# castorini/dhr

Hardware: AMD Instinct MI355X
Metric: queries/sec (exact top-1000, brute-force dense-hybrid GIP retrieval) (higher is better)
Workload: dtype i8 (bound GEMM: gated AND ungated columns int8 x int8 -> int32 on the matrix cores, every gated rounding upward, the ungated quantisation error paid by the filter margin) + f64-accumulated f16 x f32 exact rescoring of the survivors -- the returned scores are the exact scores rounded once, identical

## Files before the change

dhr_amd/csrc/gemm_g8.h:

```cpp
#pragma once
#include "gemm_common.h"
#include <climits>

namespace dhr {

typedef int intx4 __attribute__((ext_vector_type(4)));
typedef int intx8 __attribute__((ext_vector_type(8)));

constexpr int G8_QOFF = 16384;
constexpr int G8_SLOT = 32768;
constexpr int G8_META = 4 * G8_SLOT;
constexpr int G8_RING_LDS = 4 * G8_SLOT + 4096 + 64;
constexpr int G8_NT = 512;


__device__ __forceinline__ void g8_smfmac(floatx16& c, const intx4& a, const intx8& b, uint32_t idx) {
  asm("v_smfmac_i32_32x32x64_i8 %0, %1, %2, %3" : "+v"(c) : "v"(a), "v"(b), "v"(idx));
}
__device__ __forceinline__ void g8_mfma(floatx16& c, const intx4& a, const intx4& b) {
  asm("v_mfma_i32_32x32x32_i8 %0, %1, %2, %0" : "+v"(c) : "v"(a), "v"(b));
}

struct G8Frag {
  intx4 a[4];
  intx4 pw;
  union { intx8 v; intx4 h[2]; } b[2];
};

__device__ __forceinline__ int g8_thr_units(float thr, float mul) {
  const float x = thr / mul;
  if (!(x < 2.1e9f)) return INT_MAX;
  if (x < -2.1e9f) return INT_MIN;
  return (int)floorf(x - fabsf(x) * 1e-6f) - 1;
}
__device__ __forceinline__ float g8_score(int sum, float mul) {
  const float x = (float)sum * mul;
  return x + fabsf(x) * 2.4e-7f;
}


hipError_t launch_gemm_g8p(const GemmArgs& a, hipStream_t s);
bool gemm_g8p_ok(const GemmArgs& a);

}
```

dhr_amd/csrc/gemm_g8.hip:

```cpp
#include "gemm_g8.h"
#include <mutex>
#include <type_traits>

#ifndef G8_TRACE
#define G8_TRACE 0
#endif
#ifndef G8_ABL
#define G8_ABL 0
#endif
namespace dhr {

#if G8_TRACE
constexpr int G8_TRACE_SLOTS = 1 << 18;
__device__ unsigned long long g8_trace_buf[G8_TRACE_SLOTS * 8];
__device__ unsigned int g8_trace_n;
#define G8_T(i) do { if (threadIdx.x == 0 && tslot < G8_TRACE_SLOTS) g8_trace_buf[(size_t)tslot * 8 + (i)] = __builtin_readcyclecounter(); } while (0)
#else
#define G8_T(i) do { } while (0)
#endif
__device__ __forceinline__ void g8_dump_tile(const GemmArgs& p, floatx16 (&acc)[4][2], int64_t dt, int qt, int wm, int wn, int lane,
                                             const float (&mul_r)[2]) {
  const int fhalf = lane >> 5;
  const int64_t row_base = dt * TILE_ROWS + wm * 128;
#pragma unroll
  for (int ni = 0; ni < 2; ++ni) {
    const int q = qt * TILE_ROWS + wn * 64 + ni * 32 + (lane & 31);
    if (q < p.n_queries) {
#pragma unroll
      for (int mi = 0; mi < 4; ++mi)
#pragma unroll
        for (int e = 0; e < 16; ++e) {
          const int64_t row = row_base + mi * 32 + (e & 3) + 8 * (e >> 2) + 4 * fhalf;
          if (row < p.n_rows && row >= p.dump_row0 && row - p.dump_row0 < p.dump_ld)
            p.dump[(int64_t)q * p.dump_ld + (row - p.dump_row0)] = g8_score(__float_as_int(acc[mi][ni][e]), mul_r[ni]);
        }
    }
  }
}

template <bool SURPLUS, int NI_, bool CHECK_ROWS = true>
__device__ __forceinline__ void g8_scan_half(const GemmArgs& p, floatx16 (&acc)[4][2], int qt, int wm, int wn, int lane, int rows_valid, int64_t row0,
                                             uint2* stack, const int t, const float mul, uint32_t& j) {
  const int fhalf = lane >> 5;
  const int rbase = wm * 128 + 4 * fhalf;
  const int q = qt * TILE_ROWS + wn * 64 + NI_ * 32 + (lane & 31);
#pragma unroll
  for (int mi = 0; mi < 4; ++mi) {
    const floatx16& a = acc[mi][NI_];
#pragma unroll
    for (int g = 0; g < 4; ++g) {
      const int gm = max(max(__float_as_int(a[4 * g]), __float_as_int(a[4 * g + 1])), max(__float_as_int(a[4 * g + 2]), __float_as_int(a[4 * g + 3])));
      if (gm >= t) {
        asm volatile("");
        if constexpr (!SURPLUS && !CHECK_ROWS) {
#pragma unroll
          for (int e = 4 * g; e < 4 * g + 4; ++e) {
            const int v = __float_as_int(a[e]);
            const int rl = rbase + mi * 32 + (e & 3) + 8 * (e >> 2);
            const uint32_t slot = j < (uint32_t)EPI_STACK ? j : (uint32_t)EPI_STACK;
            stack[slot * G8_NT] = make_uint2((uint32_t)rl, (uint32_t)v);
            j += v >= t ? 1u : 0u;
          }
        } else
#pragma unroll
        for (int e = 4 * g; e < 4 * g + 4; ++e) {
          const int v = __float_as_int(a[e]);
          const int rl = rbase + mi * 32 + (e & 3) + 8 * (e >> 2);
          if (v >= t && (!CHECK_ROWS || rl < rows_valid)) {
            asm volatile("");
            if constexpr (SURPLUS) {
              if (j >= EPI_STACK) {
                const uint32_t slot = atomicAdd(p.cnt + q, 1u);
                cand_store(p, q, slot, make_uint2((uint32_t)(row0 + rl), __float_as_uint(g8_score(v, mul))));
              }
            } else if (j < EPI_STACK) stack[j * G8_NT] = make_uint2((uint32_t)rl, (uint32_t)v);
            ++j;
          }
        }
      }
    }
  }
}
__device__ __forceinline__ void g8_epilogue_surplus(const GemmArgs& p, floatx16 (&acc)[4][2], int qt, int wm, int wn, int lane, int rows_valid, int64_t row0,
                                                 const int (&thr_r)[2], const float (&mul_r)[2]) {
  uint32_t j = 0;
  g8_scan_half<true, 0>(p, acc, qt, wm, wn, lane, rows_valid, row0, nullptr, thr_r[0], mul_r[0], j);
  g8_scan_half<true, 1>(p, acc, qt, wm, wn, lane, rows_valid, row0, nullptr, thr_r[1], mul_r[1], j);
}
__device__ __forceinline__ void g8_epilogue(const GemmArgs& p, floatx16 (&acc)[4][2], int64_t dt, int qt, int wm, int wn, int tid, int lane,
                                            char* smem, const int (&thr_r)[2], const float (&mul_r)[2]) {
  __syncthreads();
  const int64_t row0 = dt * TILE_ROWS;
  const int rows_valid = (int)(p.n_rows - row0 < TILE_ROWS ? p.n_rows - row0 : TILE_ROWS);
  uint2* stack = (uint2*)smem + tid;
  const int q0 = qt * TILE_ROWS + wn * 64 + (lane & 31);
  const bool full = rows_valid == TILE_ROWS;
  uint32_t j = 0;
  if (full) g8_scan_half<false, 0, false>(p, acc, qt, wm, wn, lane, rows_valid, row0, stack, thr_r[0], mul_r[0], j);
  else g8_scan_half<false, 0, true>(p, acc, qt, wm, wn, lane, rows_valid, row0, stack, thr_r[0], mul_r[0], j);
  const uint32_t s0 = j < (uint32_t)EPI_STACK ? j : (uint32_t)EPI_STACK;
#if G8_ABL != 16
  uint32_t base0 = 0u, base1 = 0u;
  if (s0 > 0) base0 = atomicAdd(p.cnt + q0, s0);
#endif
  if (full) g8_scan_half<false, 1, false>(p, acc, qt, wm, wn, lane, rows_valid, row0, stack, thr_r[1], mul_r[1], j);
  else g8_scan_half<false, 1, true>(p, acc, qt, wm, wn, lane, rows_valid, row0, stack, thr_r[1], mul_r[1], j);
  const uint32_t s1 = j < (uint32_t)EPI_STACK ? j : (uint32_t)EPI_STACK;
#if G8_ABL == 16
  return;
#else
  if (s1 > s0) base1 = atomicAdd(p.cnt + q0 + 32, s1 - s0);
  if (__builtin_amdgcn_ballot_w64(j > (uint32_t)EPI_STACK) != 0) g8_epilogue_surplus(p, acc, qt, wm, wn, lane, rows_valid, row0, thr_r, mul_r);
  for (uint32_t i = 0; i < s0; ++i) {
    const uint2 en = stack[i * G8_NT];
    const uint32_t slot = base0 + i;
    cand_store(p, q0, slot, make_uint2((uint32_t)row0 + en.x, __float_as_uint(g8_score((int)en.y, mul_r[0]))));
  }
  for (uint32_t i = s0; i < s1; ++i) {
    const uint2 en = stack[i * G8_NT];
    const uint32_t slot = base1 + (i - s0);
    cand_store(p, q0 + 32, slot, make_uint2((uint32_t)row0 + en.x, __float_as_uint(g8_score((int)en.y, mul_r[1]))));
  }
#endif
}

#if G8_ABL == 2
#define G8_PAIR_SYNC() do { asm volatile("s_waitcnt lgkmcnt(0)" ::: "memory"); __builtin_amdgcn_s_barrier(); } while (0)
#elif G8_ABL == 3
#define G8_PAIR_SYNC() do { asm volatile("s_waitcnt lgkmcnt(0)" ::: "memory"); } while (0)
#else
#define G8_PAIR_SYNC() do { asm volatile("s_waitcnt vmcnt(0) lgkmcnt(0)" ::: "memory"); __builtin_amdgcn_s_barrier(); } while (0)
#endif

#ifndef G8_DMA_SCHED
#define G8_DMA_SCHED 1
#endif
#if G8_DMA_SCHED == 1
__host__ __device__ constexpr int g8_dma_piece(int ph, int g) { return ph == 0 ? g : -1; }
#elif G8_DMA_SCHED == 2
__host__ __device__ constexpr int g8_dma_piece(int ph, int g) { return ph == 0 ? (g >= 2 ? g - 2 : -1) : (ph == 1 && g < 2) ? 6 + g : -1; }
#else
__host__ __device__ constexpr int g8_dma_piece(int ph, int g) { return (ph <= 1 && (g & 1)) ? ph * 4 + (g >> 1) : -1; }
#endif

template <bool DUMP, bool PARTIAL>
__device__ __forceinline__ void g8_tile(const GemmArgs& p, char* smem, const int64_t dt, const int qt, const unsigned tslot = 0) {
  const int lane = threadIdx.x & 63;
  const int wave = __builtin_amdgcn_readfirstlane(threadIdx.x >> 6);
  const int ts = p.ts, td = p.td;
  const int nsp = ts >> 1, npairs = (ts + td) >> 1;
  const char* a_src = (const char*)p.a_tiles + dt * ((int64_t)ts * S8_STAGE_A + (int64_t)td * SP_DENSE);
  const char* b_src = (const char*)p.b_tiles + (int64_t)qt * ((int64_t)ts * SP_STAGE_B + (int64_t)td * SP_DENSE);
  const int wm = PARTIAL ? (wave & 1) : (wave >> 2), wn = PARTIAL ? (wave >> 1) : (wave & 3);
  const bool active = !PARTIAL || wn < p.partial_wn;

  const bool dma_b = ((wave >> 1) & 1) != 0;
  const int dma_s = wave >> 2;
  const int dma_h = wave & 1;
  const uint32_t lane_off = (uint32_t)lane * 16u;
  const uint32_t smem_u = (uint32_t)(uintptr_t)LDS_PTR(smem);
  const __amdgpu_buffer_rsrc_t role_rsrc = __builtin_amdgcn_make_buffer_rsrc((void*)(dma_b ? b_src : a_src), (short)0, 0x7fffffff, 0x00020000);
  int dma_soff = 0, dma_n = 0, nx_soff = 0, nx_n = 0;
  uint32_t dma_lds = 0, nx_lds = 0;
  auto dma_prepare = [&](int g) __attribute__((always_inline)) {
    const int u = 2 * g + dma_s;
    const bool sp = u < ts;
    const int half_bytes = dma_h * ((!dma_b && sp) ? S8_STAGE_A / 2 : 8192);
    if (dma_b) nx_soff = (sp ? u * SP_STAGE_B : ts * SP_STAGE_B + (u - ts) * SP_DENSE) + half_bytes;
    else nx_soff = (sp ? u * S8_STAGE_A : ts * S8_STAGE_A + (u - ts) * SP_DENSE) + half_bytes;
    nx_lds = smem_u + (uint32_t)((u & 3) * G8_SLOT + (dma_b ? G8_QOFF : 0) + half_bytes);
    nx_n = g < npairs ? ((!dma_b && sp) ? 5 : 8) : 0;
    if ((G8_ABL == 4 || G8_ABL == 8) && g >= 2) nx_n = 0;
  };
  auto dma_commit = [&]() __attribute__((always_inline)) { dma_soff = nx_soff; dma_lds = nx_lds; dma_n = nx_n; };
  auto dma_piece = [&](int j) __attribute__((always_inline)) {
    if (j < dma_n) {
      __attribute__((address_space(3))) void* l = (__attribute__((address_space(3))) void*)(uintptr_t)(dma_lds + (uint32_t)(j >> 2) * 4096u);
      const int so = dma_soff + (j >> 2) * 4096;
      switch (j & 3) {
        case 0: __builtin_amdgcn_raw_ptr_buffer_load_lds(role_rsrc, l, 16, (int)lane_off, so, 0, 0); break;
        case 1: __builtin_amdgcn_raw_ptr_buffer_load_lds(role_rsrc, l, 16, (int)lane_off, so, 1024, 0); break;
        case 2: __builtin_amdgcn_raw_ptr_buffer_load_lds(role_rsrc, l, 16, (int)lane_off, so, 2048, 0); break;
        default: __builtin_amdgcn_raw_ptr_buffer_load_lds(role_rsrc, l, 16, (int)lane_off, so, 3072, 0); break;
      }
    }
  };
  auto issue_pair = [&](int g) {
    dma_prepare(g);
    dma_commit();
#pragma unroll
    for (int j = 0; j < 8; ++j) dma_piece(j);
  };

  floatx16 acc[4][2];
  const int frow = lane & 31;
  const int fhalf = lane >> 5;
  const int swz4 = (frow >> 2) & 3;
  const int c0 = (fhalf ^ swz4) << 4, c1 = ((2 + fhalf) ^ swz4) << 4;
  const int a8_off = ((wm * 8 + fhalf) * 32 + frow) * 16;
  const int p8_off = S8_A_BYTES + ((wm * 2 + fhalf) * 32 + frow) * 16;
  const int ad_row = (wm * 128 + frow) * 64;
  const int q_row = G8_QOFF + (wn * 64 + frow) * 64;

  auto read_s8 = [&](G8Frag& f, const char* sl, int g) __attribute__((always_inline)) {
    if (g < 4) f.b[g >> 1].h[g & 1] = *(const intx4*)(sl + q_row + (g >> 1) * 2048 + ((g & 1) ? c1 : c0));
    else if (g < 8) f.a[g - 4] = *(const intx4*)(sl + a8_off + (g - 4) * 1024);
    else if (g == 8) f.pw = *(const intx4*)(sl + p8_off);
  };
  auto read_dn = [&](G8Frag& f, const char* sl, int cc, int g) __attribute__((always_inline)) {
    if (g < 2) f.b[g].h[0] = *(const intx4*)(sl + q_row + g * 2048 + cc);
    else if (g < 6) f.a[g - 2] = *(const intx4*)(sl + ad_row + (g - 2) * 2048 + cc);
  };
  auto blk_s8 = [&](const G8Frag& fc, G8Frag& fn, int un, bool do_load, auto ph_c) __attribute__((always_inline)) {
    constexpr int PH = decltype(ph_c)::value;
    const char* sl = smem + (un & 3) * G8_SLOT;
#pragma unroll
    for (int g = 0; g < 8; ++g) {
      const int ni = g >> 2, mi = g & 3;
      if (!PARTIAL || active) {
        if (do_load && G8_ABL != 8) {
          read_s8(fn, sl, g);
          if (g == 0) read_s8(fn, sl, 8);
        }
        g8_smfmac(acc[mi][ni], fc.a[mi], fc.b[ni].v, (uint32_t)fc.pw[mi]);
      }
      if (g8_dma_piece(PH, g) >= 0) dma_piece(g8_dma_piece(PH, g));
      __builtin_amdgcn_sched_barrier(0);
    }
  };
  auto blk_dn = [&](const G8Frag& fc, G8Frag& fn, int tn, bool do_load, auto ph_c) __attribute__((always_inline)) {
    constexpr int PH = decltype(ph_c)::value;
    const char* sl = smem + ((ts + (tn >> 1)) & 3) * G8_SLOT;
    const int cc = (tn & 1) ? c1 : c0;
#pragma unroll
    for (int g = 0; g < 8; ++g) {
      const int ni = g >> 2, mi = g & 3;
      if (!PARTIAL || active) {
        if (do_load && G8_ABL != 8) read_dn(fn, sl, cc, g);
        g8_mfma(acc[mi][ni], fc.a[mi], fc.b[ni].h[0]);
      }
      if (g8_dma_piece(PH, g) >= 0) dma_piece(g8_dma_piece(PH, g));
      __builtin_amdgcn_sched_barrier(0);
    }
  };

  if (wave < 4 && (ts > 0 || wave == 1 || wave == 2)) {
    const char* src = wave == 0 ? (const char*)(p.g8_rsum + dt * TILE_ROWS) : wave == 1 ? (const char*)(p.i8_mul + qt * TILE_ROWS)
                    : wave == 2 ? (const char*)(p.thr + qt * TILE_ROWS) : (const char*)(p.g8_shift + qt * TILE_ROWS);
    __builtin_amdgcn_global_load_lds(GLOBAL_PTR(src + lane_off), LDS_PTR(smem + G8_META + wave * 1024), 16, 0, 0);
  }
  issue_pair(0);
  if (npairs > 1) {
    issue_pair(1);
    if (dma_n == 5) asm volatile("s_waitcnt vmcnt(5)" ::: "memory"); else asm volatile("s_waitcnt vmcnt(8)" ::: "memory");
  } else asm volatile("s_waitcnt vmcnt(0)" ::: "memory");
  __builtin_amdgcn_s_barrier();
  G8_T(2);
  if (ts > 0) {
    const int32_t* rs = (const int32_t*)(smem + G8_META) + wm * 128 + 4 * (lane >> 5);
#pragma unroll
    for (int mi = 0; mi < 4; ++mi)
#pragma unroll
      for (int g4 = 0; g4 < 4; ++g4) {
        const intx4 v = *(const intx4*)(rs + mi * 32 + 8 * g4);
#pragma unroll
        for (int i4 = 0; i4 < 4; ++i4) acc[mi][0][4 * g4 + i4] = acc[mi][1][4 * g4 + i4] = __int_as_float(v[i4]);
      }
  } else {
#pragma unroll
    for (int mi = 0; mi < 4; ++mi)
#pragma unroll
      for (int e = 0; e < 16; ++e) acc[mi][0][e] = acc[mi][1][e] = 0.f;
  }
  int sh_r[2];
  float mul_r[2], thr_f[2];
#pragma unroll
  for (int ni = 0; ni < 2; ++ni) {
    const int ql = wn * 64 + ni * 32 + (lane & 31);
    mul_r[ni] = ((const float*)(smem + G8_META + 1024))[ql];
    thr_f[ni] = ((const float*)(smem + G8_META + 2048))[ql];
    sh_r[ni] = ts > 0 ? ((const int*)(smem + G8_META + 3072))[ql] : 0;
    asm volatile("" : "+v"(mul_r[ni]), "+v"(thr_f[ni]), "+v"(sh_r[ni]));
  }
  G8Frag f0, f1;
  if (ts > 0) {
#pragma unroll
    for (int g = 0; g < 9; ++g) read_s8(f0, smem, g);
  }
  if (G8_ABL == 8) f1 = f0;
  constexpr std::integral_constant<int, 0> PH0{};
  constexpr std::integral_constant<int, 1> PH1{};
  constexpr std::integral_constant<int, 2> PH2{};
  dma_n = 0;
#pragma unroll 1
  for (int g = 0; g + 1 < nsp; ++g) {
    blk_s8(f0, f1, 2 * g + 1, true, PH1);
    dma_prepare(g + 2);
    __builtin_amdgcn_sched_barrier(0);
    G8_PAIR_SYNC();
    dma_commit();
    blk_s8(f1, f0, 2 * g + 2, true, PH0);
  }
  if (nsp > 0) {
    const int g = nsp - 1;
    blk_s8(f0, f1, 2 * g + 1, true, PH1);
    dma_prepare(g + 2);
    __builtin_amdgcn_sched_barrier(0);
    G8_PAIR_SYNC();
    dma_commit();
    blk_s8(f1, f0, 2 * g + 2, false, PH0);
  }
  G8_T(3);
  if (td > 0) {
    __builtin_amdgcn_sched_barrier(0);
    asm volatile("s_waitcnt lgkmcnt(0)\n\ts_nop 15\n\ts_nop 7" ::: "memory");
    __builtin_amdgcn_sched_barrier(0);
    if (ts > 0)
#pragma unroll
    for (int mi = 0; mi < 4; ++mi)
#pragma unroll
      for (int ni = 0; ni < 2; ++ni)
#pragma unroll
        for (int e = 0; e < 16; ++e) acc[mi][ni][e] = __uint_as_float(__float_as_uint(acc[mi][ni][e]) << sh_r[ni]);
    __builtin_amdgcn_sched_barrier(0);
    {
      const char* sl = smem + (ts & 3) * G8_SLOT;
#pragma unroll
      for (int g = 0; g < 6; ++g) read_dn(f0, sl, c0, g);
    }
    asm volatile("s_nop 4" ::: "memory");
    __builtin_amdgcn_sched_barrier(0);
#pragma unroll 1
    for (int g = nsp; g + 1 < npairs; ++g) {
      const int t0 = 4 * (g - nsp);
      blk_dn(f0, f1, t0 + 1, true, PH1);
      blk_dn(f1, f0, t0 + 2, true, PH2);
      blk_dn(f0, f1, t0 + 3, true, PH2);
      dma_prepare(g + 2);
      __builtin_amdgcn_sched_barrier(0);
      G8_PAIR_SYNC();
      dma_commit();
      blk_dn(f1, f0, t0 + 4, true, PH0);
    }
    {
      const int g = npairs - 1;
      const int t0 = 4 * (g - nsp);
      blk_dn(f0, f1, t0 + 1, true, PH1);
      blk_dn(f1, f0, t0 + 2, true, PH2);
      blk_dn(f0, f1, t0 + 3, true, PH2);
      dma_prepare(g + 2);
      __builtin_amdgcn_sched_barrier(0);
      G8_PAIR_SYNC();
      dma_commit();
      blk_dn(f1, f0, t0 + 4, false, PH0);
    }
  }
  G8_T(4);
  asm volatile("s_waitcnt vmcnt(0) lgkmcnt(0)\n\ts_nop 15\n\ts_nop 7" ::: "memory");
  G8_T(5);
  if (DUMP) { g8_dump_tile(p, acc, dt, qt, wm, wn, lane, mul_r); return; }
  int thr_r[2];
#pragma unroll
  for (int ni = 0; ni < 2; ++ni) {
    asm volatile("" : "+v"(thr_f[ni]));
    thr_r[ni] = g8_thr_units(thr_f[ni], mul_r[ni]);
  }
#if G8_ABL == 32
  if (p.n_queries >= 0) { if (__float_as_int(acc[0][0][0]) == 0x7fffffff) p.cnt[0] = 1; return; }
#endif
  if (PARTIAL && !active) { __syncthreads(); return; }
  g8_epilogue(p, acc, dt, qt, wm, wn, (int)threadIdx.x, lane, smem, thr_r, mul_r);
}

#define G8_KERNEL_ATTR __attribute__((amdgpu_waves_per_eu(2, 2)))
template <bool DUMP>
__global__ void __launch_bounds__(G8_NT) G8_KERNEL_ATTR gemm_filter_g8_kernel(GemmArgs p) {
  extern __shared__ __attribute__((aligned(16))) char smem[];
  int64_t dt;
  int qt;
  if (!gemm_wg_tile(p, dt, qt)) return;
#if G8_TRACE
  unsigned tslot = 0;
  if (threadIdx.x == 0) tslot = atomicAdd(&g8_trace_n, 1u);
  tslot = __builtin_amdgcn_readfirstlane(tslot);
  if (threadIdx.x == 0 && tslot < G8_TRACE_SLOTS) {
    unsigned hw, xcc;
    asm volatile("s_getreg_b32 %0, hwreg(HW_REG_HW_ID)" : "=s"(hw));
    asm volatile("s_getreg_b32 %0, hwreg(HW_REG_XCC_ID)" : "=s"(xcc));
    g8_trace_buf[(size_t)tslot * 8 + 0] = __builtin_amdgcn_s_memrealtime();
    g8_trace_buf[(size_t)tslot * 8 + 7] = (unsigned long long)hw | ((unsigned long long)(xcc & 0xf) << 32) | ((unsigned long long)qt << 40) | ((unsigned long long)(dt & 0xffff) << 48);
  }
  G8_T(1);
  if (!DUMP && p.partial_wn > 0 && qt == p.n_qtiles - 1) g8_tile<false, true>(p, smem, dt, qt, tslot);
  else g8_tile<DUMP, false>(p, smem, dt, qt, tslot);
  G8_T(6);
#else
  if (!DUMP && p.partial_wn > 0 && qt == p.n_qtiles - 1) g8_tile<false, true>(p, smem, dt, qt);
  else g8_tile<DUMP, false>(p, smem, dt, qt);
#endif
}
#if G8_TRACE
}
extern "C" int dhr_debug_g8_trace(unsigned long long* out, int max_slots, unsigned* n_out) try {
  unsigned n = 0;
  if (hipMemcpyFromSymbol(&n, HIP_SYMBOL(dhr::g8_trace_n), 4) != hipSuccess) return -1;
  if (n_out) *n_out = n;
  const unsigned m = n < (unsigned)max_slots ? n : (unsigned)max_slots;
  const unsigned mm = m < (unsigned)dhr::G8_TRACE_SLOTS ? m : (unsigned)dhr::G8_TRACE_SLOTS;
  if (out && mm && hipMemcpyFromSymbol(out, HIP_SYMBOL(dhr::g8_trace_buf), (size_t)mm * 64) != hipSuccess) return -1;
  const unsigned zero = 0;
  if (hipMemcpyToSymbol(HIP_SYMBOL(dhr::g8_trace_n), &zero, 4) != hipSuccess) return -1;
  return 0;
} DHR_CATCH_STATUS
namespace dhr {
#endif

hipError_t launch_gemm_g8(const GemmArgs& a, dim3 grid, hipStream_t s) {
  static std::mutex attr_mu;
  static bool attr_set_dev[64] = {};
  int dev_ = 0;
  (void)hipGetDevice(&dev_);
  {
    std::lock_guard<std::mutex> attr_lock(attr_mu);
    bool& attr_set = attr_set_dev[dev_ & 63];
    if (!attr_set) {
      hipError_t e = hipFuncSetAttribute((const void*)gemm_filter_g8_kernel<false>, hipFuncAttributeMaxDynamicSharedMemorySize, G8_RING_LDS);
      if (e != hipSuccess) return e;
      e = hipFuncSetAttribute((const void*)gemm_filter_g8_kernel<true>, hipFuncAttributeMaxDynamicSharedMemorySize, G8_RING_LDS);
      if (e != hipSuccess) return e;
      attr_set = true;
    }
  }
  if (a.dump) { hipLaunchKernelGGL(gemm_filter_g8_kernel<true>, grid, dim3(G8_NT), G8_RING_LDS, s, a); return hipGetLastError(); }
  GemmArgs b = a;
  constexpr int partial_on = 1;
  const int valid_last = a.n_queries - (a.n_qtiles - 1) * TILE_ROWS;
  b.partial_wn = (partial_on && valid_last > 0 && valid_last <= 128) ? (valid_last + 63) / 64 : 0;
  hipLaunchKernelGGL(gemm_filter_g8_kernel<false>, grid, dim3(G8_NT), G8_RING_LDS, s, b);
  return hipGetLastError();
}

}
```

Baseline: 61680.

## Stage whole above-threshold accumulator groups in LDS with a bitmask for candidate emission

New measurement: 61970, median of 6. About the same (+0.5%).

```diff
diff --git a/dhr_amd/csrc/gemm_g8.h b/dhr_amd/csrc/gemm_g8.h
--- a/dhr_amd/csrc/gemm_g8.h
+++ b/dhr_amd/csrc/gemm_g8.h
@@ -12,6 +12,8 @@
 constexpr int G8_META = 4 * G8_SLOT;
 constexpr int G8_RING_LDS = 4 * G8_SLOT + 4096 + 64;
 constexpr int G8_NT = 512;
+constexpr int G8_GSTACK = 15;
+static_assert((G8_GSTACK + 1) * 16 * G8_NT <= 4 * G8_SLOT, "the group stacks live in the staging ring");
 
 
 __device__ __forceinline__ void g8_smfmac(floatx16& c, const intx4& a, const intx8& b, uint32_t idx) {
diff --git a/dhr_amd/csrc/gemm_g8.hip b/dhr_amd/csrc/gemm_g8.hip
--- a/dhr_amd/csrc/gemm_g8.hip
+++ b/dhr_amd/csrc/gemm_g8.hip
@@ -14,9 +14,16 @@
 constexpr int G8_TRACE_SLOTS = 1 << 18;
 __device__ unsigned long long g8_trace_buf[G8_TRACE_SLOTS * 8];
 __device__ unsigned int g8_trace_n;
-#define G8_T(i) do { if (threadIdx.x == 0 && tslot < G8_TRACE_SLOTS) g8_trace_buf[(size_t)tslot * 8 + (i)] = __builtin_readcyclecounter(); } while (0)
-#else
-#define G8_T(i) do { } while (0)
+#define G8_STAMP(i) do { if (threadIdx.x == 0 && tslot < G8_TRACE_SLOTS) g8_trace_buf[(size_t)tslot * 8 + (i)] = __builtin_readcyclecounter(); } while (0)
+#else
+#define G8_STAMP(i) do { } while (0)
+#endif
+#if G8_TRACE == 2
+#define G8_T(i) do { if ((i) != 3 && (i) != 4) G8_STAMP(i); } while (0)
+#define G8_TE(i) G8_STAMP(i)
+#else
+#define G8_T(i) G8_STAMP(i)
+#define G8_TE(i) do { } while (0)
 #endif
 __device__ __forceinline__ void g8_dump_tile(const GemmArgs& p, floatx16 (&acc)[4][2], int64_t dt, int qt, int wm, int wn, int lane,
                                              const float (&mul_r)[2]) {
@@ -38,12 +45,8 @@
   }
 }
 
-template <bool SURPLUS, int NI_, bool CHECK_ROWS = true>
-__device__ __forceinline__ void g8_scan_half(const GemmArgs& p, floatx16 (&acc)[4][2], int qt, int wm, int wn, int lane, int rows_valid, int64_t row0,
-                                             uint2* stack, const int t, const float mul, uint32_t& j) {
-  const int fhalf = lane >> 5;
-  const int rbase = wm * 128 + 4 * fhalf;
-  const int q = qt * TILE_ROWS + wn * 64 + NI_ * 32 + (lane & 31);
+template <int NI_>
+__device__ __forceinline__ void g8_scan_half(floatx16 (&acc)[4][2], intx4* stack, const int t, uint32_t& jg, uint32_t& mask) {
 #pragma unroll
   for (int mi = 0; mi < 4; ++mi) {
     const floatx16& a = acc[mi][NI_];
@@ -52,74 +55,107 @@
       const int gm = max(max(__float_as_int(a[4 * g]), __float_as_int(a[4 * g + 1])), max(__float_as_int(a[4 * g + 2]), __float_as_int(a[4 * g + 3])));
       if (gm >= t) {
         asm volatile("");
-        if constexpr (!SURPLUS && !CHECK_ROWS) {
-#pragma unroll
-          for (int e = 4 * g; e < 4 * g + 4; ++e) {
-            const int v = __float_as_int(a[e]);
-            const int rl = rbase + mi * 32 + (e & 3) + 8 * (e >> 2);
-            const uint32_t slot = j < (uint32_t)EPI_STACK ? j : (uint32_t)EPI_STACK;
-            stack[slot * G8_NT] = make_uint2((uint32_t)rl, (uint32_t)v);
-            j += v >= t ? 1u : 0u;
-          }
-        } else
-#pragma unroll
-        for (int e = 4 * g; e < 4 * g + 4; ++e) {
-          const int v = __float_as_int(a[e]);
-          const int rl = rbase + mi * 32 + (e & 3) + 8 * (e >> 2);
-          if (v >= t && (!CHECK_ROWS || rl < rows_valid)) {
-            asm volatile("");
-            if constexpr (SURPLUS) {
-              if (j >= EPI_STACK) {
-                const uint32_t slot = atomicAdd(p.cnt + q, 1u);
-                cand_store(p, q, slot, make_uint2((uint32_t)(row0 + rl), __float_as_uint(g8_score(v, mul))));
-              }
-            } else if (j < EPI_STACK) stack[j * G8_NT] = make_uint2((uint32_t)rl, (uint32_t)v);
-            ++j;
+        const uint32_t slot = jg < (uint32_t)G8_GSTACK ? jg : (uint32_t)G8_GSTACK;
+        intx4 v;
+        v[0] = __float_as_int(a[4 * g]); v[1] = __float_as_int(a[4 * g + 1]); v[2] = __float_as_int(a[4 * g + 2]); v[3] = __float_as_int(a[4 * g + 3]);
+        stack[slot * G8_NT] = v;
+        ++jg;
+        mask |= 1u << (NI_ * 16 + mi * 4 + g);
+      }
+    }
+  }
+}
+typedef uint32_t g8_u32x2 __attribute__((ext_vector_type(2)));
+__device__ __forceinline__ void g8_cand_store(const GemmArgs& p, int q, uint32_t slot, uint32_t row, uint32_t score_bits) {
+  g8_u32x2 v;
+  v[0] = row; v[1] = score_bits;
+  typedef __attribute__((address_space(1))) g8_u32x2* gptr;
+  if (slot < p.cap) *(gptr)(uintptr_t)(p.cand + (int64_t)q * p.cap + slot) = v;
+  else if (p.tier) {
+    const ListTier* t = p.tier;
+    const uint32_t o = slot - p.cap;
+    if (o < t->ovf_cap[q]) *(gptr)(uintptr_t)(t->ovf + (size_t)t->ovf_off[q] + o) = v;
+  }
+}
+__device__ __forceinline__ int g8_group_row(int b, int rbase) { return rbase + ((b >> 2) & 3) * 32 + (b & 3) * 8; }
+
+__device__ __forceinline__ void g8_epilogue_surplus(const GemmArgs& p, floatx16 (&acc)[4][2], int q0, int rbase, int rows_valid, int64_t row0,
+                                                    const int (&thr_r)[2], const float (&mul_r)[2], uint32_t mask) {
+#pragma unroll
+  for (int ni = 0; ni < 2; ++ni)
+#pragma unroll
+    for (int mi = 0; mi < 4; ++mi)
+#pragma unroll
+      for (int g = 0; g < 4; ++g) {
+        const int b = ni * 16 + mi * 4 + g;
+        if (b < G8_GSTACK) continue;
+        if (((mask >> b) & 1u) && __popc(mask & ((1u << b) - 1u)) >= G8_GSTACK) {
+#pragma unroll
+          for (int e = 0; e < 4; ++e) {
+            const int v = __float_as_int(acc[mi][ni][4 * g + e]);
+            const int rl = g8_group_row(b, rbase) + e;
+            if (v >= thr_r[ni] && rl < rows_valid) {
+              const uint32_t slot = atomicAdd(p.cnt + q0 + 32 * ni, 1u);
+              cand_store(p, q0 + 32 * ni, slot, make_uint2((uint32_t)(row0 + rl), __float_as_uint(g8_score(v, mul_r[ni]))));
+            }
           }
         }
       }
-    }
-  }
-}
-__device__ __forceinline__ void g8_epilogue_surplus(const GemmArgs& p, floatx16 (&acc)[4][2], int qt, int wm, int wn, int lane, int rows_valid, int64_t row0,
-                                                 const int (&thr_r)[2], const float (&mul_r)[2]) {
-  uint32_t j = 0;
-  g8_scan_half<true, 0>(p, acc, qt, wm, wn, lane, rows_valid, row0, nullptr, thr_r[0], mul_r[0], j);
-  g8_scan_half<true, 1>(p, acc, qt, wm, wn, lane, rows_valid, row0, nullptr, thr_r[1], mul_r[1], j);
 }
 __device__ __forceinline__ void g8_epilogue(const GemmArgs& p, floatx16 (&acc)[4][2], int64_t dt, int qt, int wm, int wn, int tid, int lane,
-                                            char* smem, const int (&thr_r)[2], const float (&mul_r)[2]) {
+                                            char* smem, const int (&thr_r)[2], const float (&mul_r)[2], const unsigned tslot) {
   __syncthreads();
   const int64_t row0 = dt * TILE_ROWS;
   const int rows_valid = (int)(p.n_rows - row0 < TILE_ROWS ? p.n_rows - row0 : TILE_ROWS);
-  uint2* stack = (uint2*)smem + tid;
+  intx4* stack = (intx4*)smem + tid;
   const int q0 = qt * TILE_ROWS + wn * 64 + (lane & 31);
-  const bool full = rows_valid == TILE_ROWS;
-  uint32_t j = 0;
-  if (full) g8_scan_half<false, 0, false>(p, acc, qt, wm, wn, lane, rows_valid, row0, stack, thr_r[0], mul_r[0], j);
-  else g8_scan_half<false, 0, true>(p, acc, qt, wm, wn, lane, rows_valid, row0, stack, thr_r[0], mul_r[0], j);
-  const uint32_t s0 = j < (uint32_t)EPI_STACK ? j : (uint32_t)EPI_STACK;
-#if G8_ABL != 16
-  uint32_t base0 = 0u, base1 = 0u;
-  if (s0 > 0) base0 = atomicAdd(p.cnt + q0, s0);
-#endif
-  if (full) g8_scan_half<false, 1, false>(p, acc, qt, wm, wn, lane, rows_valid, row0, stack, thr_r[1], mul_r[1], j);
-  else g8_scan_half<false, 1, true>(p, acc, qt, wm, wn, lane, rows_valid, row0, stack, thr_r[1], mul_r[1], j);
-  const uint32_t s1 = j < (uint32_t)EPI_STACK ? j : (uint32_t)EPI_STACK;
+  const int rbase = wm * 128 + 4 * (lane >> 5);
+  uint32_t jg = 0, mask = 0;
+  g8_scan_half<0>(acc, stack, thr_r[0], jg, mask);
+  g8_scan_half<1>(acc, stack, thr_r[1], jg, mask);
 #if G8_ABL == 16
   return;
 #else
-  if (s1 > s0) base1 = atomicAdd(p.cnt + q0 + 32, s1 - s0);
-  if (__builtin_amdgcn_ballot_w64(j > (uint32_t)EPI_STACK) != 0) g8_epilogue_surplus(p, acc, qt, wm, wn, lane, rows_valid, row0, thr_r, mul_r);
-  for (uint32_t i = 0; i < s0; ++i) {
-    const uint2 en = stack[i * G8_NT];
-    const uint32_t slot = base0 + i;
-    cand_store(p, q0, slot, make_uint2((uint32_t)row0 + en.x, __float_as_uint(g8_score((int)en.y, mul_r[0]))));
-  }
-  for (uint32_t i = s0; i < s1; ++i) {
-    const uint2 en = stack[i * G8_NT];
-    const uint32_t slot = base1 + (i - s0);
-    cand_store(p, q0 + 32, slot, make_uint2((uint32_t)row0 + en.x, __float_as_uint(g8_score((int)en.y, mul_r[1]))));
+  const uint32_t ng = jg < (uint32_t)G8_GSTACK ? jg : (uint32_t)G8_GSTACK;
+  uint32_t c0 = 0, c1 = 0;
+  {
+    uint32_t m = mask;
+    for (uint32_t k = 0; k < ng; ++k) {
+      const int b = __ffs(m) - 1;
+      m &= m - 1;
+      const intx4 v = stack[k * G8_NT];
+      const int t = b >> 4 ? thr_r[1] : thr_r[0];
+      const int rl = g8_group_row(b, rbase);
+      uint32_t n = 0;
+#pragma unroll
+      for (int e = 0; e < 4; ++e) n += (v[e] >= t && rl + e < rows_valid) ? 1u : 0u;
+      if (b >> 4) c1 += n; else c0 += n;
+    }
+  }
+  G8_TE(3);
+  uint32_t base0 = 0u, base1 = 0u;
+  if (c0 > 0) base0 = atomicAdd(p.cnt + q0, c0);
+  if (c1 > 0) base1 = atomicAdd(p.cnt + q0 + 32, c1);
+  if (__builtin_amdgcn_ballot_w64(jg > (uint32_t)G8_GSTACK) != 0) g8_epilogue_surplus(p, acc, q0, rbase, rows_valid, row0, thr_r, mul_r, mask);
+  __builtin_amdgcn_s_waitcnt(0x0f70);
+  G8_TE(4);
+  uint32_t m = mask;
+  for (uint32_t k = 0; k < ng; ++k) {
+    const int b = __ffs(m) - 1;
+    m &= m - 1;
+    const intx4 v = stack[k * G8_NT];
+    const int ni = b >> 4;
+    const int t = ni ? thr_r[1] : thr_r[0];
+    const float mul = ni ? mul_r[1] : mul_r[0];
+    const int rl = g8_group_row(b, rbase);
+    uint32_t slot = ni ? base1 : base0;
+#pragma unroll
+    for (int e = 0; e < 4; ++e)
+      if (v[e] >= t && rl + e < rows_valid) {
+        g8_cand_store(p, q0 + 32 * ni, slot, (uint32_t)(row0 + rl + e), __float_as_uint(g8_score(v[e], mul)));
+        ++slot;
+      }
+    if (ni) base1 = slot; else base0 = slot;
   }
 #endif
 }
@@ -369,7 +405,7 @@
   if (p.n_queries >= 0) { if (__float_as_int(acc[0][0][0]) == 0x7fffffff) p.cnt[0] = 1; return; }
 #endif
   if (PARTIAL && !active) { __syncthreads(); return; }
-  g8_epilogue(p, acc, dt, qt, wm, wn, (int)threadIdx.x, lane, smem, thr_r, mul_r);
+  g8_epilogue(p, acc, dt, qt, wm, wn, (int)threadIdx.x, lane, smem, thr_r, mul_r, tslot);
 }
 
 #define G8_KERNEL_ATTR __attribute__((amdgpu_waves_per_eu(2, 2)))
```
